# lssfau/ExaStencils

Measured on AMD Instinct MI355X. Metric: LU/s, higher is better.
Workload: dtype f64; 1 GPU; 3D Poisson 7-point Jacobi smoother steps (ghost exchange + sweep + advance), 512 x 512 x 512 cells per GPU, reference field layout (515-double rows); three consecutive steps per pass over HBM (temporal blocking, bit-identical); levels=9, align=0

## Files before the change

### exastencils_amd/csrc/kernels_twostage.hip

```cpp
#include "examg_common.h"

#include <type_traits>

namespace examg {

struct TSGeom {
  int ntx, nty, ntz, zc, nblocks, remap;
  int xs;
  int ys, zs;
  int first;
  Box box1;
  int ax0, ax1, ay0, ay1, az0, az1;
};

constexpr int TS_OUT = 124;

__device__ __forceinline__ long long uniform64(long long v) {
  const unsigned lo = __builtin_amdgcn_readfirstlane((unsigned)v), hi = __builtin_amdgcn_readfirstlane((unsigned)((unsigned long long)v >> 32));
  return (long long)(((unsigned long long)hi << 32) | lo);
}

struct TSProl {
  LayoutDev lc;
  const double *uc;
};

#ifndef TS_SCALAR_WV
#define TS_SCALAR_WV 1
#endif
template <int ORDER, bool COL, int NW, bool NT, int WPE, int VAR, int PF = 0, int RPW = 2, bool FMA = false>
__global__ void __launch_bounds__(64 * NW, WPE)
k_two_stage7_lds(LayoutDev lu, const double *__restrict__ u, LayoutDev lf, const double *__restrict__ rhs,
                 double *__restrict__ out, Coef7 k, double w, Box box, TSGeom g, TSProl pr) {
  constexpr bool PROL = VAR == 1, ZIN = VAR == 2;
  static_assert(RPW == 2 || VAR == 0, "the folded forms are written for two rows per wave");
  constexpr int NS = RPW * NW;
  constexpr int NI = NS + 2;
  constexpr int NO = NS - 2;
  constexpr int NCR = NI / 2 + 1, CW = 66, CT = NCR * CW;
  __shared__ d2 SM[2 * NI * 64 + 2 * NS * 64 + (PROL ? CT : 0)];
  d2 *const UBp = SM;
  d2 *const VBp = SM + 2 * NI * 64;
  double *const CBp = reinterpret_cast<double *>(SM + 2 * NI * 64 + 2 * NS * 64);
#define UB(p, i) UBp[((p) * NI + (i)) * 64 + lane]
#define VB(p, s) VBp[((p) * NS + (s)) * 64 + lane]
  const int lane = threadIdx.x, wv = TS_SCALAR_WV ? __builtin_amdgcn_readfirstlane(threadIdx.y) : threadIdx.y;
  int t = blockIdx.x;
  if (g.remap == 1) {
    const int per = g.nblocks >> 3;
    if (t < (per << 3)) t = (t & 7) * per + (t >> 3);
  } else if (g.remap == 2) {
    const int xy = g.ntx * g.nty;
    const int lz = t / xy, r = t - lz * xy;
    const int per = xy >> 3;
    t = lz * xy + (r < (per << 3) ? (r & 7) * per + (r >> 3) : r);
  }
  const int tx = t % g.ntx;
  t /= g.ntx;
  const int ty = t % g.nty;
  const int tz = t / g.nty;
  const int xw = box.b0 - 2 - g.xs + TS_OUT * tx;
  const int xa = xw + 2 * lane;
  const int rw0 = box.b1 - g.ys + ty * NO;
  const int mb = box.b2 - g.zs + tz * g.zc;
  const int mlo = max(mb, box.b2);
  const int me = min(mb + g.zc, box.e2);
  const Box &box1 = g.box1;
  const bool inx_a = xa >= box.b0 && xa < box.e0, inx_b = xa + 1 >= box.b0 && xa + 1 < box.e0;
  const bool in1_a = xa >= box1.b0 && xa < box1.e0, in1_b = xa + 1 >= box1.b0 && xa + 1 < box1.e0;
  const bool out_lane = lane >= 1 && lane <= 62;
  const bool st_a = out_lane && inx_a, st_b = out_lane && inx_b;

  const int s0 = RPW * wv;
  int grow[RPW];
  bool row_in1[RPW], row_out[RPW];
#pragma unroll
  for (int r = 0; r < RPW; ++r) {
    grow[r] = rw0 - 1 + s0 + r;
    row_in1[r] = grow[r] >= box1.b1 && grow[r] < box1.e1;
    row_out[r] = s0 + r >= 1 && s0 + r <= NS - 2 && grow[r] >= box.b1 && grow[r] < box.e1;
  }
  const bool has_outer = wv == 0 || wv == NW - 1;
  const int outer_i = wv == 0 ? 0 : NI - 1;

  struct Site {
    const char *row;
    unsigned voff;
  };
  auto site = [&](const double *base, const LayoutDev &l, int R) {
    const int rc = min(max(R + l.ref1, 0), l.tot1 - 1), i0 = xw + l.ref0;
    Site st;
    st.row = reinterpret_cast<const char *>(base + ((long long)i0 + (long long)((unsigned)l.s1 * (unsigned)rc)));
    st.voff = (unsigned)(min(max(2 * lane, -i0 - (rc == 0 ? 0 : 1)), l.tot0 - 1 - i0 - (rc == l.tot1 - 1 ? 1 : 0)) * 8);
    return st;
  };
  struct PlaneCursor {
    int p;
    long long bytes, step;
    int last;
  };
  auto cursor = [&](const LayoutDev &l, int P) {
    PlaneCursor c;
    c.p = P + l.ref2;
    c.last = l.tot2 - 1;
    c.step = uniform64(l.s2 * 8);
    c.bytes = uniform64(l.s2 * 8 * min(max(c.p, 0), c.last));
    return c;
  };
  auto advance = [&](PlaneCursor &c) {
    ++c.p;
    c.bytes += (c.p >= 1 && c.p <= c.last) ? c.step : 0LL;
  };
  auto load_at = [&](const Site &st, long long pb) {
    return load2(reinterpret_cast<const double *>(st.row + pb + st.voff));
  };
  Site urow[RPW], frow[RPW];
#pragma unroll
  for (int r = 0; r < RPW; ++r) {
    urow[r] = site(u, lu, grow[r]);
    frow[r] = site(rhs, lf, grow[r]);
  }
  const Site uouter = site(u, lu, rw0 - 2 + outer_i);
  PlaneCursor cu = cursor(lu, mb - 2), cf = cursor(lf, mb - 1);
  auto load_u = [&](const Site &st) {
    if constexpr (ZIN) return d2{0.0, 0.0};
    return load_at(st, cu.bytes);
  };
  auto load_f = [&](int r) { return load_at(frow[r], cf.bytes); };
  const unsigned vo = (unsigned)lane * 16u;
  char *obase[RPW];
#pragma unroll
  for (int r = 0; r < RPW; ++r)
    obase[r] = reinterpret_cast<char *>(out + ((long long)(xw + lu.ref0) + (long long)((unsigned)lu.s1 * (unsigned)max(grow[r] + lu.ref1, 0))));
  long long obytes = uniform64(lu.s2 * 8 * (long long)(mb - 2 + lu.ref2));
  const long long ostep = uniform64(lu.s2 * 8);

  d2 U[4][RPW], V[4][RPW], F[4][RPW], O[4];
  d2 Ocur = {0.0, 0.0};
  O[0] = O[1] = O[2] = O[3] = Ocur;
#pragma unroll
  for (int j = 0; j < 4; ++j) {
#pragma unroll
    for (int r = 0; r < RPW; ++r) U[j][r] = load_u(urow[r]);
    if (has_outer && j >= 1) {
      const d2 o = load_u(uouter);
      if (j == 1) Ocur = o;
      else O[j] = o;
    }
    advance(cu);
  }
#pragma unroll
  for (int j = 1; j < 3; ++j) {
#pragma unroll
    for (int r = 0; r < RPW; ++r) F[j][r] = load_f(r);
// ... 266 lines not shown
  const bool even = !(lu.s1 & 1) && !(lu.s2 & 1) && !(lf.s1 & 1) && !(lf.s2 & 1);
  g.xs = (even && ((lu.origin + box.b0) & 1) && ((lf.origin + box.b0) & 1)) ? 1 : 0;
  g.ys = g.zs = 0;
  if (prol) {
    g.xs = box.b0 & 1;
    g.ys = (box.b1 & 1) ? 0 : 1;
    g.zs = box.b2 & 1;
  }
  g.ntx = (box.n0() + g.xs + TS_OUT - 1) / TS_OUT;
  g.nty = (box.n1() + g.ys + NO - 1) / NO;
  const int xy = g.ntx * g.nty;
  const int n2 = box.n2() + g.zs;
  int blocks_target = 3072;
  if (prol) {
    blocks_target = xy * ((n2 + 47) / 48);
    if (blocks_target < 1536) blocks_target = 1536;
  } else if (box.count() >= 50000000LL) {
    blocks_target = 1 << 24;
  }
  const bool mid = box.count() < 50000000LL && (long long)xy * ((n2 + 15) / 16) >= 512;
  if (mid) {
    long long best = -1;
    int best_t = 1;
    for (int t = 1; t <= (n2 + 7) / 8; ++t) {
      int c = (n2 + t - 1) / t;
      if (prol || COL) c += c & 1;
      const int tt = (n2 + c - 1) / c;
      const long long cost = (((long long)xy * tt + 255) / 256) * (c + 6);
      if (best < 0 || cost < best || (cost == best && tt > best_t)) { best = cost; best_t = tt; }
    }
    blocks_target = xy * best_t;
  }
  if (g_ts_blocks > 0) blocks_target = g_ts_blocks;
  int ntz = (blocks_target + xy - 1) / xy;
  if (ntz < 1) ntz = 1;
  int zc = (n2 + ntz - 1) / ntz;
  int minzc = g_ts_minzc;
  if (minzc < 0) minzc = ((long long)xy * ((n2 + 15) / 16) < 512 || (mid && g_ts_blocks <= 0)) ? (prol ? 8 : 10) : (prol ? 16 : 14);
  if (zc < minzc) zc = minzc;
  if (g_ts_minzc < 0 && g_ts_blocks <= 0 && !prol) zc += (6 - (zc & 3)) & 3;
  if (prol || COL) zc += zc & 1;
  if (lu.s2 >= (1LL << 32) || lf.s2 >= (1LL << 32)) { set_error("examg two-stage kernel: a plane must hold less than 2^32 elements"); return 1; }
  if (zc > n2) zc = n2 + ((prol || COL) ? (n2 & 1) : 0);
  g.zc = zc;
  g.ntz = (n2 + zc - 1) / zc;
  g.nblocks = xy * g.ntz;
  g.remap = g_ts_remap >= 0 ? g_ts_remap : 2;
  g.first = first;
  g.box1 = box1;
  g.ax0 = -lu.ref0; g.ax1 = lu.tot0 - lu.ref0;
  g.ay0 = -lu.ref1; g.ay1 = lu.tot1 - lu.ref1;
  g.az0 = -lu.ref2; g.az1 = lu.tot2 - lu.ref2;
  const Coef7 k = make_coef7(st);
  const int ord = canonical_order7(st);
  dim3 block(64, NW, 1), grid(g.nblocks, 1, 1);
  TSProl pr;
  pr.lc = lu;
  pr.uc = nullptr;
  if (prol) pr = *prol;
  if (zero_in && !(COL && NW != 6)) {
    set_error("examg two-stage kernel: no zero-input variant of this form");
    return 1;
  }
  if (RPW != 2 && (prol || zero_in)) { set_error("examg two-stage kernel: the folded forms have two rows per wave"); return 1; }
  const int pf = COL ? ((box.b0 - 2 - g.xs) + (box.b1 - g.ys - 1) + (box.b2 - g.zs - 1) + first) & 1 : 0;
  const bool nt = g_ts_nt >= 0 ? g_ts_nt != 0 : box.count() * 24LL > 200000000LL;
  constexpr bool TS_FMA_FORM = !COL && NW == 8;
  const bool fma = TS_FMA_FORM && !g_pow2_fma_off && pow2_offdiag7(st);
#define EXAMG_TS_LAUNCH(ORD, W, V, PFV)                                                                                                               \
  do {                                                                                                                                                \
    if ((V) == 0 && (W) == 1 && !nt)                                                                                                                  \
      hipLaunchKernelGGL((k_two_stage7_lds<ORD, COL, NW, false, 1, 0, PFV, RPW>), grid, block, 0, s, lu, u, lf, rhs, out, k, w, box, g, pr);           \
    else if constexpr (TS_FMA_FORM && (V) == 0 && (W) == 1) {                                                                                         \
      if (fma)                                                                                                                                        \
        hipLaunchKernelGGL((k_two_stage7_lds<ORD, COL, NW, true, 1, 0, PFV, RPW, true>), grid, block, 0, s, lu, u, lf, rhs, out, k, w, box, g, pr);   \
      else                                                                                                                                            \
        hipLaunchKernelGGL((k_two_stage7_lds<ORD, COL, NW, true, 1, 0, PFV, RPW>), grid, block, 0, s, lu, u, lf, rhs, out, k, w, box, g, pr);         \
    } else                                                                                                                                            \
      hipLaunchKernelGGL((k_two_stage7_lds<ORD, COL, NW, true, W, V, PFV, ((V) == 0 ? RPW : 2)>), grid, block, 0, s, lu, u, lf, rhs, out, k, w, box, g, pr); \
  } while (0)
#define EXAMG_TS_LAUNCH_PF(ORD, W, V)              \
  do {                                             \
    if constexpr (COL) {                           \
      if (pf) EXAMG_TS_LAUNCH(ORD, W, V, 1);       \
      else EXAMG_TS_LAUNCH(ORD, W, V, 0);          \
    } else {                                       \
      EXAMG_TS_LAUNCH(ORD, W, V, 0);               \
    }                                              \
  } while (0)
#define EXAMG_TS_LAUNCH_ORD(W, V)                  \
  do {                                             \
    if (ord == 0) EXAMG_TS_LAUNCH_PF(0, W, V);     \
    else EXAMG_TS_LAUNCH_PF(1, W, V);              \
  } while (0)
  if (prol) {
    if (g_ts_prol_wpe == 4) EXAMG_TS_LAUNCH_ORD((NW == 6 ? 1 : 4), 1);
    else EXAMG_TS_LAUNCH_ORD(1, 1);
  } else if (zero_in) {
    if constexpr (COL && NW != 6) EXAMG_TS_LAUNCH_ORD(WPE, 2);
  } else {
    bool done = false;
    if constexpr (NW != 6 && RPW == 2) {
      if (g_ts_wpe == 4) {
        EXAMG_TS_LAUNCH_ORD(4, 0);
        done = true;
      }
    }
    if (!done) EXAMG_TS_LAUNCH_ORD(1, 0);
  }
#undef EXAMG_TS_LAUNCH_ORD
#undef EXAMG_TS_LAUNCH_PF
#undef EXAMG_TS_LAUNCH
  EXAMG_CHECK_LAUNCH("k_two_stage7_lds");
  return 0;
}

template <bool COL>
static int launch_two_stage(const examg_layout_t *lu_, const double *u, const examg_layout_t *lf_, const double *rhs,
                            double *out, const examg_stencil_t *st, double w, int first, const Box &box, hipStream_t s,
                            const Box *box1 = nullptr, const TSProl *prol = nullptr, bool zero_in = false) {
  const Box &b1 = box1 ? *box1 : box;
  int impl = g_ts_lds == -2 ? (box.n1() >= 192 ? 8 : 5) : g_ts_lds;
  if (zero_in && impl == 6) impl = 5;
  if (g_ts_lds == -2 && impl == 8 && !prol && !zero_in && box.count() >= 50000000LL) impl = 83;
  if (impl == 83 && !prol && !zero_in)
    return launch_two_stage_lds<COL, 8, 1, 3>(lu_, u, lf_, rhs, out, st, w, first, box, b1, s, prol, zero_in);
  if (impl == 83) impl = 8;
  if (impl == 8) return launch_two_stage_lds<COL, 8>(lu_, u, lf_, rhs, out, st, w, first, box, b1, s, prol, zero_in);
  if (impl == 6) return launch_two_stage_lds<COL, 6>(lu_, u, lf_, rhs, out, st, w, first, box, b1, s, prol, zero_in);
  return launch_two_stage_lds<COL, 5>(lu_, u, lf_, rhs, out, st, w, first, box, b1, s, prol, zero_in);
}

static bool prolong_args_ok(const char *who, const examg_layout_t *lc, const Box &box) {
  if (box.b0 < 0 || box.b1 < 0 || box.b2 < 0) { set_error("%s: negative fine index", who); return false; }
  int32_t cb[3] = {box.b0 / 2, box.b1 / 2, box.b2 / 2}, ce[3] = {box.e0 / 2 + 1, box.e1 / 2 + 1, box.e2 / 2 + 1};
  if (lc->nd != 3 || !box_inside(lc, make_box(cb, ce), 0)) { set_error("%s: coarse footprint leaves the coarse allocation", who); return false; }
  return true;
}

static bool two_stage_ok(const examg_layout_t *lu, const examg_layout_t *lf, const examg_stencil_t *st, const Box &box) {
  return !g_ts_disable && !lay_split(lu) && !lay_split(lf) && lu->nd == 3 && canonical_order7(st) >= 0 && box.n0() >= 64 && box_inside(lu, box, 1) &&
         box_inside(lf, box, 0) && make_layout(lu).s2 < (1LL << 32) && make_layout(lf).s2 < (1LL << 32);
}

static bool stage_boxes_ok(const examg_layout_t *lf_, const Box &box1, const Box &box2) {
  const LayoutDev lf = make_layout(lf_);
  const bool lo = box1.b0 < box2.b0 && box2.b1 + lf.ref1 == 0 && box2.b2 + lf.ref2 == 0;
  const bool hi = box1.e0 > box2.e0 && box2.e1 + lf.ref1 == lf.tot1 && box2.e2 + lf.ref2 == lf.tot2;
  return !lo && !hi;
}

constexpr int TS3_OUT = 120;

template <int ORDER, int NW, bool NT, int RPW = 3, bool COL = false, bool FMA = false>
__global__ void __launch_bounds__(64 * NW, 1)
k_three_stage7_lds(LayoutDev lu, const double *__restrict__ u, LayoutDev lf, const double *__restrict__ rhs,
                   double *__restrict__ out, Coef7 k, double w, Box box, TSGeom g) {
  constexpr int NS = RPW * NW;
  constexpr int NO = NS - 4;
  __shared__ d2 SM[3 * 2 * 2 * NW * 64];
#define EB(f, p, h, wq) EBW(wave_rows(wq), f, p, h)
#define EBW(rows, f, p, h) (rows)[((((f) * 2 + (p)) * 2 + (h)) * 64)]
  auto wave_rows = [&](int wq) {
    unsigned off = (unsigned)wq * (3 * 2 * 2 * 64 * 16);
    asm volatile("" : "+s"(off));
    return reinterpret_cast<d2 *>(reinterpret_cast<char *>(SM) + off + threadIdx.x * 16u);
  };
  const int lane = threadIdx.x, wv = __builtin_amdgcn_readfirstlane(threadIdx.y);
  int t = blockIdx.x;
  if (g.remap == 2) {
    const int xy = g.ntx * g.nty;
    const int lz = t / xy, r = t - lz * xy;
    const int per = xy >> 3;
    t = lz * xy + (r < (per << 3) ? (r & 7) * per + (r >> 3) : r);
  }
  const int tx = t % g.ntx;
  t /= g.ntx;
  const int ty = t % g.nty;
  const int tz = t / g.nty;
  const int xw = box.b0 - 4 + TS3_OUT * tx;
  const int xa = xw + 2 * lane;
  const int rw0 = box.b1 + ty * NO;
  const int mb = box.b2 + tz * g.zc;
  const int me = min(mb + g.zc, box.e2);
  const bool inx_a = xa >= box.b0 && xa < box.e0, inx_b = xa + 1 >= box.b0 && xa + 1 < box.e0;
  const bool out_lane = lane >= 2 && lane <= 61;
  const bool st_a = out_lane && inx_a, st_b = out_lane && inx_b;
  const int s0 = RPW * wv;
  int grow[RPW];
  bool row_in[RPW], row_out[RPW];
#pragma unroll
  for (int r = 0; r < RPW; ++r) {
    grow[r] = rw0 - 2 + s0 + r;
    row_in[r] = grow[r] >= box.b1 && grow[r] < box.e1;
    row_out[r] = s0 + r >= 2 && s0 + r <= NS - 3 && row_in[r];
  }
  const bool has_outer = wv == 0 || wv == NW - 1;
  const int outer_row = wv == 0 ? rw0 - 3 : rw0 - 2 + NS;
  const int wlo = wv >= 1 ? wv - 1 : 0, whi = wv + 1 <= NW - 1 ? wv + 1 : NW - 1;

  struct Site {
    const char *row;
    unsigned voff;
  };
  auto site = [&](const double *base, const LayoutDev &l, int R) {
    const int rc = min(max(R + l.ref1, 0), l.tot1 - 1), i0 = xw + l.ref0;
    Site st;
    st.row = reinterpret_cast<const char *>(base + ((long long)i0 + (long long)((unsigned)l.s1 * (unsigned)rc)));
    st.voff = (unsigned)(min(max(2 * lane, -i0 - (rc == 0 ? 0 : 1)), l.tot0 - 1 - i0 - (rc == l.tot1 - 1 ? 1 : 0)) * 8);
    return st;
  };
  struct PlaneCursor {
    int p;
    long long bytes, step;
    int last;
  };
  auto cursor = [&](const LayoutDev &l, int P) {
    PlaneCursor c;
    c.p = P + l.ref2;
    c.last = l.tot2 - 1;
    c.step = uniform64(l.s2 * 8);
    c.bytes = uniform64(l.s2 * 8 * min(max(c.p, 0), c.last));
    return c;
  };
  auto advance = [&](PlaneCursor &c) {
    ++c.p;
    c.bytes += (c.p >= 1 && c.p <= c.last) ? c.step : 0LL;
  };
  auto load_at = [&](const Site &st, long long pb) { return load2(reinterpret_cast<const double *>(st.row + pb + st.voff)); };
  Site urow[RPW], frow[RPW];
#pragma unroll
  for (int r = 0; r < RPW; ++r) {
    urow[r] = site(u, lu, grow[r]);
    frow[r] = site(rhs, lf, grow[r]);
  }
  const Site uouter = site(u, lu, outer_row);
  const int q0 = mb - 2;
  PlaneCursor cu = cursor(lu, q0 - 1), cf = cursor(lf, q0);
  const unsigned vo = (unsigned)lane * 16u;
  char *obase[RPW];
#pragma unroll
  for (int r = 0; r < RPW; ++r)
    obase[r] = reinterpret_cast<char *>(out + ((long long)(xw + lu.ref0) + (long long)((unsigned)lu.s1 * (unsigned)max(grow[r] + lu.ref1, 0))));
  long long obytes = uniform64(lu.s2 * 8 * (long long)(q0 - 2 + lu.ref2));
  const long long ostep = uniform64(lu.s2 * 8);

  d2 U[4][RPW], V[4][RPW], W[4][RPW], F[4][RPW], O[4];
  O[0] = O[1] = O[2] = O[3] = d2{0.0, 0.0};
#pragma unroll
  for (int j = 0; j < 4; ++j) {
#pragma unroll
    for (int r = 0; r < RPW; ++r) U[j][r] = load_at(urow[r], cu.bytes);
    if (has_outer && j >= 1) O[j] = load_at(uouter, cu.bytes);
    advance(cu);
  }
#pragma unroll
  for (int j = 1; j < 3; ++j) {
#pragma unroll
    for (int r = 0; r < RPW; ++r) F[j][r] = load_at(frow[r], cf.bytes);
    advance(cf);
  }
#pragma unroll
  for (int r = 0; r < RPW; ++r) {
    F[0][r] = F[1][r];
    F[3][r] = F[1][r];
#pragma unroll
    for (int j = 0; j < 4; ++j) {
      V[j][r] = U[0][r];
      W[j][r] = U[0][r];
    }
  }
  EB(0, 0, 0, wv) = U[1][0];
  EB(0, 0, 1, wv) = U[1][RPW - 1];
  __builtin_amdgcn_s_waitcnt(0x0F70);
  __syncthreads();

  using I0_ = std::integral_constant<int, 0>;
  using I1_ = std::integral_constant<int, 1>;
  using I2_ = std::integral_constant<int, 2>;
  using I3_ = std::integral_constant<int, 3>;
  auto jac = [&](d2 c, d2 ym, d2 yp, d2 zm, d2 zp, d2 f) {
    const double xl = lane_below0(c.y), xr = lane_above0(c.x);
    const double acc_a = conv7<ORDER, FMA>(k, c.x, xl, c.y, ym.x, yp.x, zm.x, zp.x);
    const double acc_b = conv7<ORDER, FMA>(k, c.y, c.x, xr, ym.y, yp.y, zm.y, zp.y);
    d2 n;
    n.x = c.x + w * (f.x - acc_a);
    n.y = c.y + w * (f.y - acc_b);
    return n;
  };
  auto jac_x = [&](d2 c, d2 ym, d2 yp, d2 zm, d2 zp, d2 f) {
    const double xl = lane_below0(c.y);
    const double acc = conv7<ORDER, FMA>(k, c.x, xl, c.y, ym.x, yp.x, zm.x, zp.x);
    return c.x + w * (f.x - acc);
  };
  auto jac_y = [&](d2 c, d2 ym, d2 yp, d2 zm, d2 zp, d2 f) {
    const double xr = lane_above0(c.x);
    const double acc = conv7<ORDER, FMA>(k, c.y, c.x, xr, ym.y, yp.y, zm.y, zp.y);
    return c.y + w * (f.y - acc);
  };
  auto upd = [&](bool first_point, d2 c, d2 ym, d2 yp, d2 zm, d2 zp, d2 f) {
    if constexpr (!COL) return jac(c, ym, yp, zm, zp, f);
    d2 n = c;
    if (first_point) n.x = jac_x(c, ym, yp, zm, zp, f);
    else n.y = jac_y(c, ym, yp, zm, zp, f);
    return n;
  };
  const int cpar = xw + g.first;
  auto step = [&](const int q, auto PHc) {
    constexpr int PH = decltype(PHc)::value;
    d2 (&Um)[RPW] = U[PH & 3], (&Uc)[RPW] = U[(PH + 1) & 3], (&Up)[RPW] = U[(PH + 2) & 3];
    d2 (&Vmm)[RPW] = V[(PH + 3) & 3], (&Vm)[RPW] = V[PH & 3], (&Vn)[RPW] = V[(PH + 1) & 3];
    d2 (&Wmm)[RPW] = W[(PH + 2) & 3], (&Wm)[RPW] = W[(PH + 3) & 3], (&Wn)[RPW] = W[PH & 3];
    d2 (&Fq)[RPW] = F[(PH + 1) & 3], (&Fm)[RPW] = F[PH & 3], (&Fmm)[RPW] = F[(PH + 3) & 3];
    constexpr int ub = PH & 1, vb = (PH + 1) & 1;
    const d2 *const below = wave_rows(wlo), *const above = wave_rows(whi);
    d2 ulo = EBW(below, 0, ub, 1), uhi = EBW(above, 0, ub, 0);
    const d2 vlo = EBW(below, 1, vb, 1), vhi = EBW(above, 1, vb, 0);
    const d2 zlo = EBW(below, 2, vb, 1), zhi = EBW(above, 2, vb, 0);
    if (wv == 0) ulo = O[(PH + 1) & 3];
    if (wv == NW - 1) uhi = O[(PH + 1) & 3];
    const bool pin1 = q >= box.b2 && q < box.e2, pin2 = q - 1 >= box.b2 && q - 1 < box.e2;
    const bool run2 = q >= mb;
    const bool run3 = q - 2 >= mb && q - 2 < me;
    bool fp[RPW];
#pragma unroll
    for (int r = 0; r < RPW; ++r) fp[r] = ((cpar + grow[r] + q) & 1) == 0;
    auto stage1 = [&](auto Rc) {
      constexpr int r = decltype(Rc)::value;
      const d2 c = Uc[r];
      const d2 n = upd(fp[r], c, r == 0 ? ulo : Uc[r == 0 ? 0 : r - 1], r == RPW - 1 ? uhi : Uc[r == RPW - 1 ? r : r + 1], Um[r], Up[r], Fq[r]);
      const bool on = pin1 && row_in[r];
      Vn[r].x = (inx_a && on) ? n.x : c.x;
      Vn[r].y = (inx_b && on) ? n.y : c.y;
    };
    auto stage2 = [&](auto Rc) {
      constexpr int r = decltype(Rc)::value;
      if (run2) {
        const d2 c = Vm[r];
        const d2 n = upd(fp[r], c, r == 0 ? vlo : Vm[r == 0 ? 0 : r - 1], r == RPW - 1 ? vhi : Vm[r == RPW - 1 ? r : r + 1], Vmm[r], Vn[r], Fm[r]);
        const bool on = pin2 && row_in[r];
        Wn[r].x = (inx_a && on) ? n.x : c.x;
        Wn[r].y = (inx_b && on) ? n.y : c.y;
      }
    };
    auto stage3 = [&](auto Rc) {
      constexpr int r = decltype(Rc)::value;
      if (run3 && row_out[r]) {
        const d2 c = Wm[r];
        const d2 o = upd(fp[r], c, r == 0 ? zlo : Wm[r == 0 ? 0 : r - 1], r == RPW - 1 ? zhi : Wm[r == RPW - 1 ? r : r + 1], Wmm[r], Wn[r], Fmm[r]);
        double *qp = reinterpret_cast<double *>(obase[r] + obytes + vo);
        if (st_a && st_b) {
          if (NT) store2_nt(qp, o);
          else store2(qp, o);
        } else if (st_a) {
          qp[0] = o.x;
        } else if (st_b) {
          qp[1] = o.y;
        }
      }
    };
    if constexpr (RPW == 3) {
      stage1(I1_{});
      stage2(I1_{});
      stage3(I1_{});
      stage1(I0_{});
      stage1(I2_{});
      stage2(I0_{});
      stage2(I2_{});
      stage3(I0_{});
      stage3(I2_{});
    } else {
      stage1(I0_{});
      stage1(I1_{});
      stage2(I0_{});
      stage2(I1_{});
      stage3(I0_{});
      stage3(I1_{});
    }
    if (q <= me) {
      d2 *const own = wave_rows(wv);
      EBW(own, 0, vb, 0) = Up[0];
      EBW(own, 0, vb, 1) = Up[RPW - 1];
      EBW(own, 1, ub, 0) = Vn[0];
      EBW(own, 1, ub, 1) = Vn[RPW - 1];
      EBW(own, 2, ub, 0) = Wn[0];
      EBW(own, 2, ub, 1) = Wn[RPW - 1];
    }
#pragma unroll
    for (int r = 0; r < RPW; ++r) {
      Um[r] = load_at(urow[r], cu.bytes);
      Fmm[r] = load_at(frow[r], cf.bytes);
    }
    if (has_outer) O[PH & 3] = load_at(uouter, cu.bytes);
    advance(cu);
    advance(cf);
    obytes += ostep;
    __syncthreads();
#ifndef TS3_NO_SCHED_BARRIER
    __builtin_amdgcn_sched_barrier(0);
#endif
  };
  const int qe = me + 1;
  for (int q = q0; q <= qe; q += 4) {
    step(q, I0_{});
    step(q + 1, I1_{});
    step(q + 2, I2_{});
    step(q + 3, I3_{});
  }
#undef EB
#undef EBW
}

static thread_local int g_ts3_zc = -1;
static thread_local int g_ts3_disable = 0;
static thread_local long long g_ts3_minpts = 8000000LL;

static bool three_stage_ok(const examg_layout_t *lu, const examg_layout_t *lf, const examg_stencil_t *st, const Box &box) {
  return !g_ts3_disable && two_stage_ok(lu, lf, st, box) && box.n1() >= 20 && box.count() >= g_ts3_minpts;
}

template <int NW, int RPW, bool COL>
static int launch_three_stage_shape(const examg_layout_t *lu_, const double *u, const examg_layout_t *lf_, const double *rhs, double *out,
                                    const examg_stencil_t *st, double w, const Box &box, hipStream_t s, int first) {
  constexpr int NO = RPW * NW - 4;
  const LayoutDev lu = make_layout(lu_), lf = make_layout(lf_);
  TSGeom g;
  g.xs = g.ys = g.zs = 0;
  g.ntx = (box.n0() + TS3_OUT - 1) / TS3_OUT;
  g.nty = (box.n1() + NO - 1) / NO;
  const int xy = g.ntx * g.nty, n2 = box.n2();
  const bool fma = !COL && !g_pow2_fma_off && pow2_offdiag7(st);
  const int cmax = (fma && box.count() >= 100000000LL) ? 28 : 64;
  int zc = n2;
  {
    long long best = -1;
    for (int t = 1; t <= (n2 + 7) / 8; ++t) {
      const int c = (n2 + t - 1) / t, tt = (n2 + c - 1) / c;
      if ((c > cmax && t < (n2 + 7) / 8) || (c < 16 && t > 1)) continue;
      const long long cost = (((long long)xy * tt + 255) / 256) * (((c + 4 + 3) & ~3) + 4);
      if (best < 0 || cost < best) { best = cost; zc = c; }
    }
    if (zc + 3 < n2) zc = (zc + 3) & ~3;
  }
  if (g_ts3_zc > 0) zc = g_ts3_zc;
  if (zc > n2) zc = n2;
  g.zc = zc;
  g.ntz = (n2 + zc - 1) / zc;
  g.nblocks = xy * g.ntz;
  g.remap = g_ts_remap >= 0 ? g_ts_remap : 2;
  g.first = first;
  g.box1 = box;
  g.ax0 = -lu.ref0; g.ax1 = lu.tot0 - lu.ref0;
  g.ay0 = -lu.ref1; g.ay1 = lu.tot1 - lu.ref1;
  g.az0 = -lu.ref2; g.az1 = lu.tot2 - lu.ref2;
  const Coef7 k = make_coef7(st);
  const int ord = canonical_order7(st);
  const bool nt = g_ts_nt >= 0 ? g_ts_nt != 0 : box.count() * 24LL > 200000000LL;
  dim3 block(64, NW, 1), grid(g.nblocks, 1, 1);
  with_order(ord, [&](auto O) {
    constexpr int ORD = decltype(O)::value;
    auto go = [&](auto NTc, auto Fc) {
      hipLaunchKernelGGL((k_three_stage7_lds<ORD, NW, decltype(NTc)::value, RPW, COL, decltype(Fc)::value>), grid, block, 0, s, lu, u, lf, rhs, out, k, w, box, g);
    };
    if constexpr (!COL) {
      if (fma) return nt ? go(std::true_type{}, std::true_type{}) : go(std::false_type{}, std::true_type{});
    }
    return nt ? go(std::true_type{}, std::false_type{}) : go(std::false_type{}, std::false_type{});
  });
  EXAMG_CHECK_LAUNCH("k_three_stage7_lds");
  return 0;
}

static int launch_three_stage(const examg_layout_t *lu, const double *u, const examg_layout_t *lf, const double *rhs, double *out,
                              const examg_stencil_t *st, double w, const Box &box, hipStream_t s) {
  return launch_three_stage_shape<8, 3, false>(lu, u, lf, rhs, out, st, w, box, s, 0);
}

static int launch_three_colours(const examg_layout_t *lu, const double *u, const examg_layout_t *lf, const double *rhs, double *out,
                                const examg_stencil_t *st, double w, int first, const Box &box, hipStream_t s) {
  return launch_three_stage_shape<8, 3, true>(lu, u, lf, rhs, out, st, w, box, s, first);
}

}

using namespace examg;

#ifdef EXAMG_DEBUG_HOOKS
extern "C" int examg_debug_two_stage_lds(int nw) {
  g_ts_lds = nw < 0 ? -2 : nw;
  return 0;
}

extern "C" int examg_debug_two_stage_nt(int nt) {
  g_ts_nt = nt < 0 ? -1 : (nt ? 1 : 0);
  return 0;
}

extern "C" int examg_debug_two_stage_prol(int wpe) {
  if (wpe >= 10) g_ts_wpe = wpe - 10 == 4 ? 4 : 1;
  else g_ts_prol_wpe = wpe == 1 ? 1 : 4;
  return 0;
}

extern "C" int examg_debug_three_stage(int disable, int zc) {
  g_ts3_disable = disable == 1;
  g_ts3_minpts = disable == 2 ? (1LL << 20) : 8000000LL;
  g_ts3_zc = zc > 0 ? zc : -1;
  return 0;
}

extern "C" int examg_debug_pow2_fma(int on) {
  g_pow2_fma_off = on ? 0 : 1;
  return 0;
}

extern "C" int examg_debug_two_stage(int disable, int blocks, int remap, int wy) {
  g_ts_disable = disable;
  if (blocks != 0) g_ts_blocks = blocks > 0 ? blocks : -1;
  if (remap >= 0) g_ts_remap = remap;
  g_ts_minzc = wy > 0 ? wy : -1;
  return 0;
}
#endif

enum Route { ROUTE_NONE = 0, ROUTE_LDS, ROUTE_SMALL };

static Route two_stage_route(const examg_layout_t *lu, const examg_layout_t *lf, const examg_stencil_t *st, const Box &box1, const Box &box2) {
  if (box2.count() == 0 || !box1.contains(box2)) return ROUTE_NONE;
  if (two_stage_ok(lu, lf, st, box2) && box_inside(lu, box1, 1) && box_inside(lf, box1, 0) && stage_boxes_ok(lf, box1, box2)) return ROUTE_LDS;
  if (box1 == box2 && small_two_stage_ok(lu, lf, st, box2)) return ROUTE_SMALL;
  return ROUTE_NONE;
}

template <bool COL>
static int launch_route(Route r, const char *who, const examg_layout_t *lu, const double *u_in, double *u_out, const examg_layout_t *lf,
                        const double *rhs, const examg_stencil_t *st, double w, int first, const Box &box1, const Box &box2, int var,
                        const examg_layout_t *lc, const double *uc, hipStream_t s) {
  if (var == 1 && !prolong_args_ok(who, lc, box2)) return 1;
  if (r == ROUTE_SMALL) return launch_small_two_stage(COL, var, lu, u_in, u_out, lf, rhs, st, w, first, box2, lc, uc, s);
  TSProl pr;
  if (var == 1) pr = TSProl{make_layout(lc), uc};
  return launch_two_stage<COL>(lu, var == 2 ? u_out : u_in, lf, rhs, u_out, st, w, first, box2, s, &box1, var == 1 ? &pr : nullptr, var == 2);
}

static bool args_ok(const char *who, bool given, const void *u_in, const void *u_out, int first) {
  if (!given) { set_error("%s: null argument", who); return false; }
  if (u_in == u_out) { set_error("%s: out of place only", who); return false; }
  if (first != 0 && first != 1) { set_error("%s: first colour must be 0 or 1", who); return false; }
  return true;
}

static bool tmp_ok(const char *who, const void *tmp, const void *u_in, const void *u_out) {
  if (!tmp || tmp == u_in || tmp == u_out) { set_error("%s: fallback needs a distinct tmp array", who); return false; }
  return true;
}

static int colour_loops_on_copy(const examg_layout_t *lu, const double *u_in, double *u_out, const examg_layout_t *lc, const double *uc,
                                const examg_layout_t *lf, const double *rhs, const examg_stencil_t *st, double w, int first, int n,
                                const int32_t *begin, const int32_t *end, examg_stream_t stream) {
  int32_t gb[3], ge[3];
  grow_box(begin, end, stencil_reach(st), lu->nd, gb, ge);
  int rc = u_in ? examg_axpby(lu, u_in, lu, u_out, 1.0, 0.0, gb, ge, stream) : examg_set(lu, u_out, 0.0, gb, ge, stream);
  if (!rc && uc) rc = examg_prolong_add(lc, uc, lu, u_out, begin, end, stream);
  for (int k = 0; k < n && !rc; ++k) rc = examg_rbgs_colour(lu, u_out, lf, rhs, st, w, (k & 1) ? 1 - first : first, begin, end, stream);
  return rc;
}

static int jacobi_through_tmp(const examg_layout_t *lu, const double *u_in, double *u_out, double *tmp, const examg_layout_t *lf,
                              const double *rhs, const examg_stencil_t *st, double w, const int32_t *begin1, const int32_t *end1,
                              const int32_t *begin2, const int32_t *end2, examg_stream_t stream) {
  int32_t gb[3], ge[3];
  grow_box(begin1, end1, stencil_reach(st), lu->nd, gb, ge);
  int rc = examg_axpby(lu, u_in, lu, tmp, 1.0, 0.0, gb, ge, stream);
  if (!rc) rc = examg_jacobi(lu, u_in, tmp, lf, rhs, st, w, begin1, end1, stream);
  if (!rc && u_out) rc = examg_jacobi(lu, tmp, u_out, lf, rhs, st, w, begin2, end2, stream);
  return rc;
}

extern "C" int examg_two_stage_eligible(const examg_layout_t *lu, const examg_layout_t *lf, const examg_stencil_t *st,
                                        const int32_t *begin1, const int32_t *end1, const int32_t *begin2, const int32_t *end2) {
  if (!lu || !lf || !st || !begin1 || !end1 || !begin2 || !end2) return 0;
  return two_stage_route(lu, lf, st, make_box(begin1, end1), make_box(begin2, end2)) != ROUTE_NONE;
}

extern "C" int examg_rbgs_sweep_fused(const examg_layout_t *lu, const double *u_in, double *u_out,
                                      const examg_layout_t *lf, const double *rhs, const examg_stencil_t *st, double w,
                                      int first, const int32_t *begin, const int32_t *end, examg_stream_t stream) {
  const char *who = "examg_rbgs_sweep_fused";
  if (!args_ok(who, lu && u_in && u_out && lf && rhs && st && begin && end, u_in, u_out, first)) return 1;
  const Box box = make_box(begin, end);
  if (box.count() == 0) return 0;
  if (const Route r = two_stage_route(lu, lf, st, box, box))
    return launch_route<true>(r, who, lu, u_in, u_out, lf, rhs, st, w, first, box, box, 0, nullptr, nullptr, (hipStream_t)stream);
  return colour_loops_on_copy(lu, u_in, u_out, nullptr, nullptr, lf, rhs, st, w, first, 2, begin, end, stream);
}

extern "C" int examg_rbgs_sweep_fused_zero(const examg_layout_t *lu, double *u_out, const examg_layout_t *lf, const double *rhs,
                                           const examg_stencil_t *st, double w, int first, const int32_t *begin,
                                           const int32_t *end, examg_stream_t stream) {
  const char *who = "examg_rbgs_sweep_fused_zero";
  if (!args_ok(who, lu && u_out && lf && rhs && st && begin && end, nullptr, u_out, first)) return 1;
  const Box box = make_box(begin, end);
  if (box.count() == 0) return 0;
  if (const Route r = two_stage_route(lu, lf, st, box, box))
    return launch_route<true>(r, who, lu, nullptr, u_out, lf, rhs, st, w, first, box, box, 2, nullptr, nullptr, (hipStream_t)stream);
  return colour_loops_on_copy(lu, nullptr, u_out, nullptr, nullptr, lf, rhs, st, w, first, 2, begin, end, stream);
}

extern "C" int examg_rbgs_sweep_fused_prolong(const examg_layout_t *lu, const double *u_in, double *u_out,
                                              const examg_layout_t *lf, const double *rhs, const examg_stencil_t *st, double w,
                                              int first, const int32_t *begin, const int32_t *end, const examg_layout_t *lc,
                                              const double *uc, examg_stream_t stream) {
  const char *who = "examg_rbgs_sweep_fused_prolong";
  if (!args_ok(who, lu && u_in && u_out && lf && rhs && st && begin && end && lc && uc, u_in, u_out, first)) return 1;
  const Box box = make_box(begin, end);
  if (box.count() == 0) return 0;
  if (const Route r = two_stage_route(lu, lf, st, box, box))
    return launch_route<true>(r, who, lu, u_in, u_out, lf, rhs, st, w, first, box, box, 1, lc, uc, (hipStream_t)stream);
  return colour_loops_on_copy(lu, u_in, u_out, lc, uc, lf, rhs, st, w, first, 2, begin, end, stream);
}

extern "C" int examg_rbgs_sweep_fused_boxes(const examg_layout_t *lu, const double *u_in, double *u_out, double *tmp,
                                            const examg_layout_t *lf, const double *rhs, const examg_stencil_t *st, double w,
                                            int first, const int32_t *begin1, const int32_t *end1, const int32_t *begin2,
                                            const int32_t *end2, examg_stream_t stream) {
  const char *who = "examg_rbgs_sweep_fused_boxes";
  if (!args_ok(who, lu && u_in && u_out && lf && rhs && st && begin1 && end1 && begin2 && end2, u_in, u_out, first)) return 1;
  const Box box1 = make_box(begin1, end1), box2 = make_box(begin2, end2);
  if (box2.count() == 0) return 0;
  if (!box1.contains(box2)) { set_error("%s: the second box must lie inside the first", who); return 1; }
  if (const Route r = two_stage_route(lu, lf, st, box1, box2))
    return launch_route<true>(r, who, lu, u_in, u_out, lf, rhs, st, w, first, box1, box2, 0, nullptr, nullptr, (hipStream_t)stream);
  if (!tmp_ok(who, tmp, u_in, u_out)) return 1;
  int32_t gb[3], ge[3];
  grow_box(begin1, end1, stencil_reach(st), lu->nd, gb, ge);
  int rc = examg_axpby(lu, u_in, lu, tmp, 1.0, 0.0, gb, ge, stream);
  if (!rc) rc = examg_rbgs_colour(lu, tmp, lf, rhs, st, w, first, begin1, end1, stream);
  if (!rc) rc = examg_axpby(lu, tmp, lu, u_out, 1.0, 0.0, begin2, end2, stream);
  if (!rc) rc = examg_stencil_op(EXAMG_SMOOTH, lu, tmp, lf, rhs, lu, u_out, st, w, 1 - first, begin2, end2, stream);
  return rc;
}

static int jacobi2_boxes(const char *who, const examg_layout_t *lu, const double *u_in, double *u_out, double *tmp, const examg_layout_t *lf,
                         const double *rhs, const examg_stencil_t *st, double w, const int32_t *begin1, const int32_t *end1,
                         const int32_t *begin2, const int32_t *end2, examg_stream_t stream) {
  if (!args_ok(who, lu && u_in && u_out && lf && rhs && st && begin1 && end1 && begin2 && end2, u_in, u_out, 0)) return 1;
  const Box box1 = make_box(begin1, end1), box2 = make_box(begin2, end2);
  if (box2.count() == 0) return 0;
  if (!box1.contains(box2)) { set_error("%s: the stage-2 box must lie inside the stage-1 box", who); return 1; }
  if (const Route r = two_stage_route(lu, lf, st, box1, box2))
    return launch_route<false>(r, who, lu, u_in, u_out, lf, rhs, st, w, 0, box1, box2, 0, nullptr, nullptr, (hipStream_t)stream);
  if (const int r27 = sf27_jacobi2_try(lu, u_in, u_out, lf, rhs, st, w, box1, box2, (hipStream_t)stream)) return r27 < 0 ? 1 : 0;
  if (!tmp_ok(who, tmp, u_in, u_out)) return 1;
  return jacobi_through_tmp(lu, u_in, u_out, tmp, lf, rhs, st, w, begin1, end1, begin2, end2, stream);
}

extern "C" int examg_jacobi2_boxes(const examg_layout_t *lu, const double *u_in, double *u_out, double *tmp,
                                   const examg_layout_t *lf, const double *rhs, const examg_stencil_t *st, double w,
                                   const int32_t *begin1, const int32_t *end1, const int32_t *begin2, const int32_t *end2,
                                   examg_stream_t stream) {
// ... 70 lines not shown
```

Baseline: 620.3 billion LU/s.

## Add CU-aware segmented z-chunk plan for three-stage temporal-blocked sweep

Adds a small host-side planner that divides blocks into up to three segments, each with its own column range, z-chunk size and optional interleaved layer order. The aim is to match whole rounds of blocks to the device's CU count, queried at runtime, instead of using a fixed uniform chunk sized against 256. For large FMA or colour grids, it uses a larger chunk for most columns and tiny chunks for the few leftover columns whenever its cost model predicts fewer wave-rounds. The trade-off is longer z-chunks, which shrink halo overhead but raise per-block latency and tail risk, plus a small decode cost per block.

Measured after the change: 643.1 billion LU/s, median of 6. +3.7%, better.

```diff
diff --git a/exastencils_amd/csrc/kernels_twostage.hip b/exastencils_amd/csrc/kernels_twostage.hip
--- a/exastencils_amd/csrc/kernels_twostage.hip
+++ b/exastencils_amd/csrc/kernels_twostage.hip
@@ -1,5 +1,7 @@
 #include "examg_common.h"
-
+#include "ts3_plan.h"
+
+#include <atomic>
 #include <type_traits>
 
 namespace examg {
@@ -572,10 +574,10 @@
 
 constexpr int TS3_OUT = 120;
 
-template <int ORDER, int NW, bool NT, int RPW = 3, bool COL = false, bool FMA = false>
+template <int ORDER, int NW, bool NT, int RPW = 3, bool COL = false, bool FMA = false, bool PLAN = false>
 __global__ void __launch_bounds__(64 * NW, 1)
 k_three_stage7_lds(LayoutDev lu, const double *__restrict__ u, LayoutDev lf, const double *__restrict__ rhs,
-                   double *__restrict__ out, Coef7 k, double w, Box box, TSGeom g) {
+                   double *__restrict__ out, Coef7 k, double w, Box box, TSGeom g, TS3Plan pl) {
   constexpr int NS = RPW * NW;
   constexpr int NO = NS - 4;
   __shared__ d2 SM[3 * 2 * 2 * NW * 64];
@@ -587,22 +589,41 @@
     return reinterpret_cast<d2 *>(reinterpret_cast<char *>(SM) + off + threadIdx.x * 16u);
   };
   const int lane = threadIdx.x, wv = __builtin_amdgcn_readfirstlane(threadIdx.y);
-  int t = blockIdx.x;
-  if (g.remap == 2) {
-    const int xy = g.ntx * g.nty;
-    const int lz = t / xy, r = t - lz * xy;
-    const int per = xy >> 3;
-    t = lz * xy + (r < (per << 3) ? (r & 7) * per + (r >> 3) : r);
-  }
-  const int tx = t % g.ntx;
-  t /= g.ntx;
-  const int ty = t % g.nty;
-  const int tz = t / g.nty;
+  int t = blockIdx.x, tx, ty, mb, me;
+  if constexpr (PLAN) {
+    TS3Seg sg = pl.seg[0];
+    if (t >= pl.seg[1].first) sg = pl.seg[1];
+    if (t >= pl.seg[2].first) sg = pl.seg[2];
+    t -= sg.first;
+    const int pos = t / sg.ncol;
+    int col = t - pos * sg.ncol;
+    if (g.remap == 2) {
+      const int per = sg.ncol >> 3;
+      col = col < (per << 3) ? (col & 7) * per + (col >> 3) : col;
+    }
+    col += sg.col0;
+    const int tz = sg.order == TS3_INTERLEAVED ? ((pos & 1) ? ((sg.nl + 1) >> 1) + (pos >> 1) : (pos >> 1)) : pos;
+    ty = col / g.ntx;
+    tx = col - ty * g.ntx;
+    mb = box.b2 + sg.z0 + tz * sg.zc;
+    me = min(mb + sg.zc, box.b2 + sg.z1);
+  } else {
+    if (g.remap == 2) {
+      const int xy = g.ntx * g.nty;
+      const int lz = t / xy, r = t - lz * xy;
+      const int per = xy >> 3;
+      t = lz * xy + (r < (per << 3) ? (r & 7) * per + (r >> 3) : r);
+    }
+    tx = t % g.ntx;
+    t /= g.ntx;
+    ty = t % g.nty;
+    const int tz = t / g.nty;
+    mb = box.b2 + tz * g.zc;
+    me = min(mb + g.zc, box.e2);
+  }
   const int xw = box.b0 - 4 + TS3_OUT * tx;
   const int xa = xw + 2 * lane;
   const int rw0 = box.b1 + ty * NO;
-  const int mb = box.b2 + tz * g.zc;
-  const int me = min(mb + g.zc, box.e2);
   const bool inx_a = xa >= box.b0 && xa < box.e0, inx_b = xa + 1 >= box.b0 && xa + 1 < box.e0;
   const bool out_lane = lane >= 2 && lane <= 61;
   const bool st_a = out_lane && inx_a, st_b = out_lane && inx_b;
@@ -833,6 +854,21 @@
 
 static thread_local int g_ts3_zc = -1;
 static thread_local int g_ts3_disable = 0;
+static thread_local int g_ts3_m = 0, g_ts3_rounds = 0, g_ts3_order = -1, g_ts3_cus = 0;
+constexpr int TS3_ROUNDS_CMAX = 256;
+constexpr int TS3_ROUNDS_ORDER = TS3_NATURAL;
+
+static int device_cus() {
+  static std::atomic<int> cus[64];
+  int dev = 0;
+  if (hipGetDevice(&dev) != hipSuccess || dev < 0 || dev >= 64) return 256;
+  int n = cus[dev].load(std::memory_order_relaxed);
+  if (n <= 0) {
+    if (hipDeviceGetAttribute(&n, hipDeviceAttributeMultiprocessorCount, dev) != hipSuccess || n <= 0) n = 256;
+    cus[dev].store(n, std::memory_order_relaxed);
+  }
+  return n;
+}
 static thread_local long long g_ts3_minpts = 8000000LL;
 
 static bool three_stage_ok(const examg_layout_t *lu, const examg_layout_t *lf, const examg_stencil_t *st, const Box &box) {
@@ -851,22 +887,19 @@
   const int xy = g.ntx * g.nty, n2 = box.n2();
   const bool fma = !COL && !g_pow2_fma_off && pow2_offdiag7(st);
   const int cmax = (fma && box.count() >= 100000000LL) ? 28 : 64;
-  int zc = n2;
-  {
-    long long best = -1;
-    for (int t = 1; t <= (n2 + 7) / 8; ++t) {
-      const int c = (n2 + t - 1) / t, tt = (n2 + c - 1) / c;
-      if ((c > cmax && t < (n2 + 7) / 8) || (c < 16 && t > 1)) continue;
-      const long long cost = (((long long)xy * tt + 255) / 256) * (((c + 4 + 3) & ~3) + 4);
-      if (best < 0 || cost < best) { best = cost; zc = c; }
-    }
-    if (zc + 3 < n2) zc = (zc + 3) & ~3;
-  }
-  if (g_ts3_zc > 0) zc = g_ts3_zc;
-  if (zc > n2) zc = n2;
-  g.zc = zc;
-  g.ntz = (n2 + zc - 1) / zc;
-  g.nblocks = xy * g.ntz;
+  TS3Rule rule;
+  rule.P = g_ts3_cus > 0 ? g_ts3_cus : device_cus();
+  rule.cmax = cmax;
+  rule.rounds_cmax = ((fma || COL) && box.count() >= 100000000LL) ? TS3_ROUNDS_CMAX : 0;
+  rule.order = g_ts3_order >= 0 ? g_ts3_order : TS3_ROUNDS_ORDER;
+  rule.force_zc = g_ts3_zc;
+  rule.force_m = g_ts3_m;
+  rule.force_rounds = g_ts3_rounds;
+  const TS3Plan pl = ts3_plan(xy, n2, rule);
+  g.zc = pl.seg[0].zc;
+  g.ntz = pl.seg[0].nl;
+  g.nblocks = pl.nblocks;
+  const bool planned = pl.nseg > 1 || pl.seg[0].order != TS3_NATURAL;
   g.remap = g_ts_remap >= 0 ? g_ts_remap : 2;
   g.first = first;
   g.box1 = box;
@@ -880,7 +913,10 @@
   with_order(ord, [&](auto O) {
     constexpr int ORD = decltype(O)::value;
     auto go = [&](auto NTc, auto Fc) {
-      hipLaunchKernelGGL((k_three_stage7_lds<ORD, NW, decltype(NTc)::value, RPW, COL, decltype(Fc)::value>), grid, block, 0, s, lu, u, lf, rhs, out, k, w, box, g);
+      if (planned)
+        hipLaunchKernelGGL((k_three_stage7_lds<ORD, NW, decltype(NTc)::value, RPW, COL, decltype(Fc)::value, true>), grid, block, 0, s, lu, u, lf, rhs, out, k, w, box, g, pl);
+      else
+        hipLaunchKernelGGL((k_three_stage7_lds<ORD, NW, decltype(NTc)::value, RPW, COL, decltype(Fc)::value, false>), grid, block, 0, s, lu, u, lf, rhs, out, k, w, box, g, pl);
     };
     if constexpr (!COL) {
       if (fma) return nt ? go(std::true_type{}, std::true_type{}) : go(std::false_type{}, std::true_type{});
@@ -926,6 +962,14 @@
   g_ts3_disable = disable == 1;
   g_ts3_minpts = disable == 2 ? (1LL << 20) : 8000000LL;
   g_ts3_zc = zc > 0 ? zc : -1;
+  return 0;
+}
+
+extern "C" int examg_debug_three_stage_plan(int layers_per_round, int rounds, int order, int cus) {
+  g_ts3_m = layers_per_round > 0 ? layers_per_round : 0;
+  g_ts3_rounds = rounds > 0 ? rounds : 0;
+  g_ts3_order = order < 0 ? -1 : (order ? TS3_INTERLEAVED : TS3_NATURAL);
+  g_ts3_cus = cus > 0 ? cus : 0;
   return 0;
 }
 
diff --git a/exastencils_amd/csrc/ts3_plan.h b/exastencils_amd/csrc/ts3_plan.h
--- /dev/null
+++ b/exastencils_amd/csrc/ts3_plan.h
@@ -0,0 +1,149 @@
+#pragma once
+
+namespace examg {
+
+constexpr int TS3_MAX_SEG = 3;
+constexpr int TS3_NATURAL = 0, TS3_INTERLEAVED = 1;
+
+struct TS3Seg {
+  int col0, ncol;
+  int z0, z1;
+  int zc;
+  int nl;
+  int first;
+  int order;
+};
+
+struct TS3Plan {
+  int nseg, nblocks;
+  TS3Seg seg[TS3_MAX_SEG];
+};
+
+inline int ts3_chunk_cost(int zc) { return ((zc + 7) & ~3) + 4; }
+
+inline int ts3_layer_at(const TS3Seg &s, int p) {
+  if (s.order != TS3_INTERLEAVED) return p;
+  return (p & 1) ? (s.nl + 1) / 2 + (p >> 1) : (p >> 1);
+}
+
+inline void ts3_plan_clear(TS3Plan &pl) {
+  pl.nseg = 0;
+  pl.nblocks = 0;
+  for (int i = 0; i < TS3_MAX_SEG; ++i) pl.seg[i] = TS3Seg{0, 0, 0, 0, 4, 0, 0, TS3_NATURAL};
+}
+
+inline void ts3_plan_add(TS3Plan &pl, int col0, int ncol, int z0, int z1, int zc, int order) {
+  if (ncol <= 0 || z1 <= z0 || pl.nseg >= TS3_MAX_SEG) return;
+  if (zc < 1) zc = 1;
+  if (zc > z1 - z0) zc = z1 - z0;
+  TS3Seg &s = pl.seg[pl.nseg++];
+  s.col0 = col0; s.ncol = ncol; s.z0 = z0; s.z1 = z1; s.zc = zc;
+  s.nl = (z1 - z0 + zc - 1) / zc;
+  s.first = pl.nblocks;
+  s.order = s.nl > 2 ? order : TS3_NATURAL;
+  pl.nblocks += ncol * s.nl;
+}
+
+inline void ts3_plan_close(TS3Plan &pl) {
+  for (int i = pl.nseg; i < TS3_MAX_SEG; ++i) pl.seg[i].first = pl.nblocks;
+}
+
+inline TS3Plan ts3_plan_uniform(int C, int planes, int zc) {
+  TS3Plan pl;
+  ts3_plan_clear(pl);
+  ts3_plan_add(pl, 0, C, 0, planes, zc, TS3_NATURAL);
+  ts3_plan_close(pl);
+  return pl;
+}
+
+inline int ts3_uniform_zc(int C, int planes, int P, int cmax, long long *cost_out = nullptr) {
+  int zc = planes;
+  long long best = -1;
+  for (int t = 1; t <= (planes + 7) / 8; ++t) {
+    const int c = (planes + t - 1) / t, tt = (planes + c - 1) / c;
+    if ((c > cmax && t < (planes + 7) / 8) || (c < 16 && t > 1)) continue;
+    const long long cost = (((long long)C * tt + P - 1) / P) * ts3_chunk_cost(c);
+    if (best < 0 || cost < best) { best = cost; zc = c; }
+  }
+  if (zc + 3 < planes) zc = (zc + 3) & ~3;
+  if (cost_out) *cost_out = best;
+  return zc;
+}
+
+inline int ts3_layers_per_round(int C, int P) {
+  if (C < 1 || P < 1) return 0;
+  int m = 1;
+  while (P / m > C) ++m;
+  return m;
+}
+
+inline TS3Plan ts3_plan_rounds(int C, int planes, int P, int m, int R, int order) {
+  TS3Plan pl;
+  ts3_plan_clear(pl);
+  if (m < 1) m = 1;
+  if (R < 1) R = 1;
+  int cm = P / m;
+  if (cm < 1) cm = 1;
+  if (cm > C) cm = C;
+  const int k = m * R;
+  int zc = ((planes + k - 1) / k + 3) & ~3;
+  ts3_plan_add(pl, 0, cm, 0, planes, zc, order);
+  const int left = C - cm;
+  if (left > 0) {
+    const int per_col = (P + left - 1) / left;
+    int lzc = ((planes + per_col - 1) / per_col + 3) & ~3;
+    if (lzc < 4) lzc = 4;
+    ts3_plan_add(pl, cm, left, 0, planes, lzc, TS3_NATURAL);
+  }
+  ts3_plan_close(pl);
+  return pl;
+}
+
+inline long long ts3_plan_cost(const TS3Plan &pl, int P) {
+  long long cost = 0;
+  for (int i = 0; i < pl.nseg; ++i)
+    cost += (((long long)pl.seg[i].ncol * pl.seg[i].nl + P - 1) / P) * ts3_chunk_cost(pl.seg[i].zc);
+  return cost;
+}
+
+inline int ts3_best_rounds(int C, int planes, int P, int m, int minzc, int cmax, long long *cost_out = nullptr) {
+  int bestR = 0;
+  long long best = -1;
+  for (int R = 1; R * m <= (planes + 3) / 4; ++R) {
+    const TS3Plan pl = ts3_plan_rounds(C, planes, P, m, R, TS3_NATURAL);
+    const int zc = pl.seg[0].zc;
+    if (zc > cmax) continue;
+    if (zc < minzc && R > 1) break;
+    const long long cost = ts3_plan_cost(pl, P);
+    if (best < 0 || cost < best) { best = cost; bestR = R; }
+  }
+  if (cost_out) *cost_out = best;
+  return bestR;
+}
+
+struct TS3Rule {
+  int P;
+  int cmax;
+  int rounds_cmax;
+  int order;
+  int force_zc;
+  int force_m, force_rounds;
+};
+
+inline TS3Plan ts3_plan(int C, int planes, const TS3Rule &r) {
+  if (r.force_zc > 0) return ts3_plan_uniform(C, planes, r.force_zc < planes ? r.force_zc : planes);
+  const int P = r.P > 0 ? r.P : 1;
+  const bool forced = r.force_m > 0 || r.force_rounds > 0;
+  long long ucost = 0;
+  const int uzc = ts3_uniform_zc(C, planes, P, r.cmax, &ucost);
+  const int m = r.force_m > 0 ? r.force_m : ts3_layers_per_round(C, P);
+  const bool few_left = m > 0 && (long long)(C - (P / m < C ? P / m : C)) * 16 <= C;
+  if (m > 0 && (forced || (r.rounds_cmax > 0 && few_left))) {
+    long long rcost = 0;
+    const int R = r.force_rounds > 0 ? r.force_rounds : ts3_best_rounds(C, planes, P, m, 16, forced && r.rounds_cmax <= 0 ? planes : r.rounds_cmax, &rcost);
+    if (R > 0 && (forced || rcost < ucost)) return ts3_plan_rounds(C, planes, P, m, R, r.order);
+  }
+  return ts3_plan_uniform(C, planes, uzc);
+}
+
+}
```
